# nebula-beta/MonocularSfM

Hardware: AMD Instinct MI355X
Metric: descriptor-pairs/sec (and image-pairs/sec); match-index bit-parity vs CPU (higher is better)
Workload: dtype f32

## Files before the change

monocularsfm_amd/csrc/msfm_batch.hip.h:

```cpp
#pragma once
namespace {
struct Batch {
    std::vector<PairDesc> pairs;
    std::vector<PfPair> pf;
    std::vector<int> id1, id2;
    std::vector<int> item_base;
    size_t n_items = 0, items_per_xcd = 0;
    MsfmItemChunks chunks = {};
    long long rp_elems = 0, cp_elems = 0, kf_elems = 0, kr_elems = 0, out_elems = 0, cand_elems = 0;
    int max_npad = 0;
    int64_t desc_pairs = 0;
    int64_t algo_bytes = 0;
    MsfmRoute route;
    std::vector<CandList> dense_lists;
    std::vector<VerifyPair> verify_pairs;
};

void build_items(Batch& b, int path, const std::vector<char>* only = nullptr, std::vector<int>* base_out = nullptr,
                 MsfmItemChunks* chunks_out = nullptr, const std::vector<char>* idle = nullptr) {
    std::vector<int> order(b.pairs.size());
    for (size_t p = 0; p < order.size(); ++p) order[p] = (int)p;
    if (b.id2.size() == b.pairs.size())
        std::stable_sort(order.begin(), order.end(), [&](int x, int y) { return b.id2[(size_t)x] < b.id2[(size_t)y]; });
    std::vector<int>& base = base_out ? *base_out : b.item_base;
// ... 367 lines not shown

constexpr size_t kTotalsBytes = 160;
constexpr int kTotalsSweep2 = 8, kTotalsSpans = 16, kTotalsSweep1 = 24, kTotalsSweep1b = 32;
struct PrefilterLaunch {
    msfm_ctx* ctx;
    Batch& b;
    size_t ev_base;
    PruneParams prune;
    size_t P = 0;
    HostClock hc;
    const MsfmRoute& route;
    std::vector<PfPair> pfq, pf16;
    long long dense_cand = 0;
    std::vector<int> item_base16;
    MsfmItemChunks chunks16 = {};
    size_t per16 = 0;
    long long kn = 1;
    hipEvent_t e0 = nullptr, e1 = nullptr, e2 = nullptr, e3 = nullptr;
    dim3 block, mgrid;
    unsigned sweep_grid = 8;
    const PairDesc* dp = nullptr;
    const PfPair* dpf = nullptr;
    float* tuv = nullptr;
    unsigned* colmask = nullptr;
    size_t n_lists = 0;
    const CandList* dl = nullptr;
    CompactPlan cp;
    size_t G = 0, M = 0;
    long long rows_cap = 0, cand_cap = 0, items_cap = 0;
    const PlanPair* dpp = nullptr;
    PlanCounts pc = {};
    PlanOut po = {};

    PrefilterLaunch(msfm_ctx* c, Batch& batch, size_t ev, PruneParams pr) : ctx(c), b(batch), ev_base(ev), prune(pr), route(batch.route) {}

    int apply_route() {
        P = b.pairs.size();
        hc = HostClock();
        SC.pf_pending = PfPending{};
        assign_partials(b, 1, 4 * ctx->cu_count);
        SC.prof.demoted_pairs += route.demoted_pairs;
        SC.pf_pending.refine = route.kind == kRouteQ8Refine;
        dense_cand = 0;
        for (size_t p = 0; p < P; ++p) {
            b.pf[p].tu_off = b.pairs[p].kf_off;
            b.pf[p].tv_off = b.pairs[p].kr_off;
            b.pf[p].cand_off = 0;
            b.pf[p].cand_cap = 0;
            if (!route.compact() && b.pairs[p].valid && b.pf[p].use) {
                b.pf[p].cand_off = dense_cand;
                b.pf[p].cand_cap = 16 * (b.pairs[p].n1 + b.pairs[p].n2) + 2048;
                dense_cand += b.pf[p].cand_cap;
                SC.pf_pending.dense_swept += (long long)b.pairs[p].n1pad * b.pairs[p].n2;
            }
        }
        pfq.clear(), pf16.clear();
        if (route.q8()) pfq = b.pf;
        for (size_t p = 0; p < P && (route.kind == kRouteI8 || route.q8()); ++p) {
            if (!b.pairs[p].valid || !b.pf[p].use) continue;
            PfPair& pp = route.q8() ? pfq[p] : b.pf[p];
            pp.use = route.q8() ? route.twin[p] : 1;
            if (!pp.use) continue;
            const Image &ia = ctx->images[b.id1[p]], &ib = ctx->images[b.id2[p]];
            pp.i8 = 1;
            if (route.q8()) {
                pp.a_h = reinterpret_cast<const _Float16*>(ia.q8);
                pp.b_h = reinterpret_cast<const _Float16*>(ib.q8);
// ... 334 lines not shown
                           SC.d_items.as<WorkItem>(), (float*)nullptr, (float*)nullptr, (float*)nullptr, (float*)nullptr,
                           (const float*)tuv, (const float*)tuv, SC.d_cand.as<int2>(), SC.d_cand_count.as<unsigned long long>(),
                           (const int*)nullptr, (int)b.n_items, (int*)nullptr, MsfmItemChunks{});
        HIPCHK(ctx, hipGetLastError());
        DBGSYNC(ctx, "sweep_kernel<2>");
        SC.prof.sweep2_launches += 1;
        HIPCHK(ctx, hipEventRecord(e3, SC.stream));
        HIPCHK(ctx, hipEventRecord(SC.sweep2_done, SC.stream));
        SC.sweep2_recorded = true;
        dl = SC.d_lists.as<CandList>();
        return MSFM_OK;
    }

    int launch_exact_and_finalize() {
        if (n_lists > 0) {
            const int wgs_per_xcd = std::max(1, ctx->cu_count / 8) * 8;
            const dim3 cgrid((unsigned)(8 * wgs_per_xcd));
            const unsigned long long* dcount = SC.d_cand_count.as<unsigned long long>();
#define MSFM_LAUNCH_EXACT(O)                                                                                             \
        hipLaunchKernelGGL(pf_exact_candidates_kernel<O>, cgrid, dim3(kExSpan), 0, SC.stream, dp, dl, dcount,                  \
                           (const int2*)SC.d_cand.as<int2>(), SC.d_best.as<unsigned long long>(), SC.d_second.as<unsigned long long>(), \
                           (int)n_lists, SC.d_totals.as<int>() + kTotalsSpans, (const int*)SC.d_cand_val.as<int>(), 0)
            if (route.kind == kRouteI8) MSFM_LAUNCH_EXACT(4);
            else if (ctx->order == MSFM_ORDER_SSE4X4) MSFM_LAUNCH_EXACT(0);
            else if (ctx->order == MSFM_ORDER_AVX2_FMA) MSFM_LAUNCH_EXACT(1);
            else MSFM_LAUNCH_EXACT(3);
#undef MSFM_LAUNCH_EXACT
            HIPCHK(ctx, hipGetLastError());
            DBGSYNC(ctx, "pf_exact_candidates_kernel");
    }
    if (!SC.keys_epilogue) {
        hipLaunchKernelGGL(pf_finalize_kernel, mgrid, dim3(256), 0, SC.stream, dp, dpf, (const float*)tuv, SC.d_best.as<unsigned long long>(),
                           SC.d_second.as<unsigned long long>(), SC.d_k_i0.as<int>(), SC.d_k_d0.as<float>(),
                           SC.d_k_d1.as<float>(), SC.d_fix_count.as<int>(), SC.d_fix_list.as<int4>(), SC.fix_cap_eff);
        HIPCHK(ctx, hipGetLastError());
        DBGSYNC(ctx, "pf_finalize_kernel");
    }
    if (n_lists > 0) {
        hipLaunchKernelGGL(pf_overflow_kernel, dim3((unsigned)((n_lists + 255) / 256)), dim3(256), 0, SC.stream, dl, (int)n_lists,
                           (const unsigned long long*)SC.d_cand_count.as<unsigned long long>(), (const PlanGroup*)SC.d_groups.as<PlanGroup>(),
                           (const int*)SC.d_gmembers.as<int>(), (const int*)SC.d_member_pair.as<int>(),
                           SC.d_overflow.as<unsigned char>(), SC.d_totals.as<unsigned long long>());
        HIPCHK(ctx, hipGetLastError());
    }
    SC.pf_pending.active = true;
    SC.pf_pending.n_lists = n_lists;
    SC.pf_pending.P = P;
    SC.pf_pending.ev_base = ev_base;
    hc.lap("launch sweep 2 .. finalize");
    return MSFM_OK;
    }

    int run() {
        int rc = apply_route();
        if (rc != MSFM_OK) return rc;
        rc = build_and_upload();
        if (rc != MSFM_OK || b.n_items == 0) return rc;
        rc = launch_sweep1();
        if (rc != MSFM_OK) return rc;
        if (route.compact()) {
            rc = plan_buffers();
            if (rc == MSFM_OK && route.q8()) rc = launch_route_q();
            if (rc == MSFM_OK) rc = launch_compact_sweep2();
        } else {
            rc = launch_dense_sweep2();
        }
        if (rc != MSFM_OK) return rc;
// ... 259 lines not shown
```

monocularsfm_amd/csrc/msfm_hostutil.h:

```cpp
#pragma once
#include <vector>

#if defined(__HIPCC__)
#include <hip/hip_runtime.h>
#define MSFM_HD __host__ __device__ inline __attribute__((always_inline))
#else
#define MSFM_HD inline
#endif

MSFM_HD int msfm_cp_pack(int hi, bool hi_valid, int lo, bool lo_valid) {
    unsigned c = 255u;
    if (lo_valid) {
        const unsigned x = (unsigned)(hi - lo) + 16u;
        int e = 27 - __builtin_clz(x);
        unsigned m = (x + (1u << e) - 1u) >> e;
        e += (int)(m >> 5);
        m = (m >> 5) ? 16u : m;
        const unsigned code = ((unsigned)e << 4) | (m - 16u);
        c = code >= 255u ? 255u : code;
    }
    return hi_valid ? (int)(((unsigned)hi << 8) | c) : (int)0x80000000;
}
constexpr int kCpNone = -(1 << 23);
MSFM_HD int msfm_cp_hi(int code) { return code >> 8; }
MSFM_HD bool msfm_cp_has_second(int code) { return (code & 255) != 255; }
MSFM_HD int msfm_cp_gap(int code) { const int c = code & 255; return ((16 + (c & 15)) << (c >> 4)) - 16; }

inline std::vector<long long> msfm_pipeline_marks(long long total, long long n_sub, double taper) {
    std::vector<long long> marks;
    if (n_sub < 2) return marks;
    const double last = taper, first = 2.0 - last;
    double acc = 0.0;
    marks.push_back(0);
// ... 192 lines not shown
    const long long rows_min = (hinted ? h_rows + h_rows / 8 : prior) + slack;
    MsfmPlanRoom r;
    r.hinted = hinted;
    r.rows = have_rows >= rows_min ? have_rows : mx(h_rows + h_rows / 2, prior) + slack;
    const long long cand_min = mx(8 * rows_min + 2048 * groups, h_cand);
    r.cand = have_cand >= cand_min ? have_cand : mx(8 * r.rows + 2048 * groups, h_cand);
    const long long items_min = mx(2 * ((rows_min / wg_rows + groups) * max_ranges + 64) / 8 * 8, (h_items + 64) / 8 * 8);
    r.items = have_items >= items_min ? have_items : mx(2 * ((r.rows / wg_rows + groups) * max_ranges + 64) / 8 * 8, (h_items + 64) / 8 * 8);
    return r;
}

inline unsigned long long msfm_pinned_piece_end(unsigned long long off) {
    const unsigned long long piece = 32ull << 20;
    if (off >= piece) return (off / piece + 1) * piece;
    unsigned long long end = 1ull << 20;
    while (end <= off) end *= 2;
    return end;
}

template <class AtomicMin>
MSFM_HD void msfm_fold_key(unsigned long long* best, unsigned long long* second, unsigned long long key, unsigned long long seen_best,
                           unsigned long long seen_second, AtomicMin amin) {
    if (key == seen_best) return;
    unsigned long long loser = key;
    if (key < seen_best) {
        const unsigned long long old = amin(best, key);
        if (old == key) return;
        loser = old > key ? old : key;
        if (loser == ~0ull) return;
    }
    if (loser < seen_second) (void)amin(second, loser);
}

MSFM_HD bool msfm_select_homography(int n_epipolar, int n_homography, double h_ratio) {
    return n_epipolar > 0 && (double)n_homography >= h_ratio * (double)n_epipolar;
}

MSFM_HD bool msfm_initial_candidate(int n_triangulated, double median_tri_angle, double mean_tri_angle, double mean_residual,
                                    int min_num_inliers, double tri_max_error, double tri_min_angle) {
    return n_triangulated >= min_num_inliers && median_tri_angle >= tri_min_angle && mean_tri_angle >= tri_min_angle &&
           mean_residual <= tri_max_error;
}
```

monocularsfm_amd/csrc/msfm_job.hip.h:

```cpp
#pragma once

static int call_prologue(msfm_ctx* ctx) {
    HIPCHK(ctx, hipSetDevice(ctx->device));
    ctx->cur = &ctx->sc[0];
    for (Scratch& s : ctx->sc) forget_sweeps(ctx, s);
    if (!ctx->deferred.empty()) {
        HIPCHK(ctx, hipDeviceSynchronize());
        ctx->deferred.flush();
    }
    return settle_store(ctx);
}

template <class Attempt>
static int rerun_alone(msfm_ctx* ctx, Attempt attempt) {
    for (int k = 1;; ++k) {
        bool retry = false;
        const int rc = attempt(&retry);
        if (rc != MSFM_OK || !retry) return rc;
        if (k >= 6) return fail(ctx, MSFM_E_DEVICE, "batch kept overflowing its queues");
    }
}

struct MatchJob {
    msfm_ctx* ctx = nullptr;
// ... 151 lines not shown
            w.b.pairs.push_back(pd);
            w.b.pf.push_back(pp);
            w.b.id1.push_back(pairs[2 * end]);
            w.b.id2.push_back(pairs[2 * end + 1]);
            ++end;
        }
        w.end = end;
        cost_done = cost_begin + cost;
        return prepare_batch_images(ctx, w.b, prune);
    }

    int issue(SubBatch& w, size_t ev_base) {
        Batch& b = w.b;
        const size_t P = b.pairs.size();
        const int begin = w.begin;
        w.ev_base = ev_base;
        w.exact_launched = false;
        SC.prof = msfm_profile{};
        SC.seq = ctx->issue_seq++;
        SC.sweep2_recorded = false;
        int rc = run_knn(ctx, b, ev_base, &w.exact_launched, prune, need_fix, true);
        if (rc != MSFM_OK) return rc;
        const long long oe = std::max<long long>(1, b.out_elems);
        HIPCHK(ctx, SC.d_st_qt.ensure(oe * sizeof(int2)));
        HIPCHK(ctx, SC.d_st_d.ensure(oe * 4));
        HIPCHK(ctx, SC.d_sub_qt.ensure(oe * sizeof(int2)));
        HIPCHK(ctx, SC.d_sub_d.ensure(oe * 4));
        HIPCHK(ctx, SC.d_counts.ensure(P * 4));
        HIPCHK(ctx, SC.d_sens.ensure(P * 4));
        HIPCHK(ctx, SC.d_offsets.ensure((P + 1) * 8));
        EpiParams ep = {prm.ratio, prm.cross_check, prm.max_distance};
        if (SC.keys_epilogue)
            hipLaunchKernelGGL(epilogue_kernel<KnnFromKeys>, dim3((unsigned)P), dim3(256), 0, SC.stream, SC.d_pairs.as<PairDesc>(), ep,
                               KnnFromKeys{SC.d_tu.as<float>(), SC.d_best.as<unsigned long long>(), SC.d_second.as<unsigned long long>()},
                               SC.d_st_qt.as<int2>(), SC.d_st_d.as<float>(), SC.d_counts.as<int>(), SC.d_sens.as<int>());
        else
            hipLaunchKernelGGL(epilogue_kernel<KnnFromArrays>, dim3((unsigned)P), dim3(256), 0, SC.stream, SC.d_pairs.as<PairDesc>(), ep,
                               KnnFromArrays{SC.d_k_i0.as<int>(), SC.d_k_d0.as<float>(), SC.d_k_d1.as<float>()},
                               SC.d_st_qt.as<int2>(), SC.d_st_d.as<float>(), SC.d_counts.as<int>(), SC.d_sens.as<int>());
        HIPCHK(ctx, hipGetLastError());
        const int* d_counts = SC.d_counts.as<int>();
        const int2* d_st_qt = SC.d_st_qt.as<int2>();
        const float* d_st_d = SC.d_st_d.as<float>();
        if (verify) {
            rc = issue_verify(b, begin, oe, ev_base);
            if (rc != MSFM_OK) return rc;
            d_counts = SC.d_counts2.as<int>();
            d_st_qt = SC.d_st2_qt.as<int2>();
            d_st_d = SC.d_st2_d.as<float>();
        }
        hipLaunchKernelGGL(scan_counts_kernel, dim3(1), dim3(256), 0, SC.stream, d_counts,
                           SC.d_offsets.as<long long>(), (int)P);
        HIPCHK(ctx, hipGetLastError());
        hipLaunchKernelGGL(gather_kernel, dim3((unsigned)P), dim3(256), 0, SC.stream, SC.d_pairs.as<PairDesc>(),
                           d_counts, SC.d_offsets.as<long long>(), d_st_qt,
                           d_st_d, SC.d_sub_qt.as<int2>(), SC.d_sub_d.as<float>());
        HIPCHK(ctx, hipGetLastError());
        rc = queue_tail_copies(ctx, P, select ? &SC.d_vs_records : nullptr);
        if (rc != MSFM_OK) return rc;
        if (pose) {
            HIPCHK(ctx, SC.h_tv.ensure(P * sizeof(msfm_two_view_record) + 64, 0));
            char* h = nullptr;
            HIPCHK(ctx, hipHostGetDevicePointer((void**)&h, SC.h_tv.p, 0));
            ExportSegs segs = {};
            segs.s[0] = ExportSeg{SC.d_tv_records.as<char>(), h, (unsigned)(P * sizeof(msfm_two_view_record))};
            hipLaunchKernelGGL(export_tail_kernel, dim3(32), dim3(256), 0, SC.stream, segs);
            HIPCHK(ctx, hipGetLastError());
// ... 372 lines not shown
```

monocularsfm_amd/csrc/msfm_kernels.hip.h:

```cpp
#pragma once
#include <hip/hip_runtime.h>
#include <stdint.h>

#pragma clang fp contract(off)

namespace msfm {

constexpr int kDim = 128;
constexpr int kBM = 128;
constexpr int kBN = 128;
constexpr int kTM = 8;
constexpr int kTN = 4;
constexpr int kThreads = 512;
constexpr int kChunkPos = 32;
constexpr int kChunks = kDim / kChunkPos;
constexpr int kPanelFloats = kBM * kDim;
constexpr int kSlotFloats = kChunkPos * kBN;
constexpr int kWaveCols = kBN / 8;
constexpr int kWaveSlotFloats = kChunkPos * kWaveCols;
constexpr int kLdsA = 0;
constexpr int kLdsB = kPanelFloats;
constexpr int kLdsFloats = kLdsB + 8 * 2 * kWaveSlotFloats;
constexpr int kLdsBytes = kLdsFloats * 4;

constexpr int kLdsBytesIdxStash = kLdsBytes + kTM * kThreads * 4;
template <int ORDER> struct OrderTraits;
template <> struct OrderTraits<0> {
    static constexpr int kGroups = 4, kIters = 8, kGroupPos = 32;
    static constexpr bool kFused = false;
    __host__ __device__ static int pos_to_k(int pos) {
        const int g = pos >> 5, v = (pos >> 3) & 3, it = pos & 7;
        const int lane = (g == 0) ? 0 : (g == 1) ? 2 : (g == 2) ? 1 : 3;
        return 16 * it + 4 * v + lane;
    }
};
// ... 417 lines not shown
template <int ORDER>
__global__ void tie_fixup_kernel(const PairDesc* __restrict__ pairs, const int* __restrict__ fix_count,
                                 const int4* __restrict__ fix_list, int fix_cap,
                                 int* __restrict__ k_i0, const float* __restrict__ k_d0) {
    MSFM_TAIL_PRIO();
    const int nfix = min(*fix_count, fix_cap);
    for (int f = blockIdx.x; f < nfix; f += gridDim.x) {
        const int4 w = fix_list[f];
        const PairDesc pd = pairs[w.x];
        const bool fwd = (w.y == 0);
        const float* me = (fwd ? pd.a_rawp : pd.b_rawp) + (size_t)w.z * kDim;
        const float* other = fwd ? pd.b_rawp : pd.a_rawp;
        const int n_other = fwd ? pd.n2 : pd.n1;
        const long long ko = (fwd ? pd.kf_off : pd.kr_off) + w.z;
        const float d0 = k_d0[ko];
        int best = 0x7fffffff;
        for (int t = threadIdx.x; t < n_other; t += 64) {
            const float s = fwd ? l2sqr_rowmajor<ORDER>(me, other + (size_t)t * kDim)
                                : l2sqr_rowmajor<ORDER>(other + (size_t)t * kDim, me);
            if (sqrtf(s) == d0) { best = t; break; }
        }
#pragma unroll
        for (int m = 32; m >= 1; m >>= 1) best = min(best, __shfl_xor(best, m));
        if (threadIdx.x == 0 && best != 0x7fffffff) k_i0[ko] = best;
    }
}

struct EpiParams {
    float ratio;
    int cross_check;
    double max_distance;
};

constexpr double kOrderEps = 1.0e-5;

__device__ __forceinline__ bool order_sensitive(int i0, float d0, float d1, float ratio, double max_distance, bool forward) {
    if (i0 < 0 || !(d1 < 3.402823466e+38f)) return false;
    const double lo0 = (double)d0 * (1.0 - kOrderEps), hi0 = (double)d0 * (1.0 + kOrderEps);
    const double lo1 = (double)d1 * (1.0 - kOrderEps), hi1 = (double)d1 * (1.0 + kOrderEps);
    if (forward && lo0 > max_distance) return false;
    const bool pass = d0 < ratio * d1;
    bool certified;
    if (pass)
        certified = hi0 < (double)ratio * lo1 && hi0 < lo1 && (!forward || hi0 <= max_distance || lo0 > max_distance);
    else
        certified = lo0 >= (double)ratio * hi1;
    return !certified;
}

struct KnnFromArrays {
    const int* i0;
    const float* d0;
    const float* d1;
    __device__ __forceinline__ void get(long long slot, int& i, float& a, float& b) const {
        i = i0[slot];
        a = d0[slot];
        b = d1[slot];
    }
};
struct KnnFromKeys {
    const float* tuv;
    const unsigned long long* best;
    const unsigned long long* second;
    __device__ __forceinline__ void get(long long slot, int& i, float& a, float& b) const {
        i = -1;
        a = b = 3.402823466e+38f;
        if (tuv[slot] == -f_inf()) return;
        const unsigned long long kb = best[slot], ks = second[slot];
        if (kb != ~0ull) { i = (int)(unsigned)(kb & 0xffffffffu); a = sqrtf(__uint_as_float((unsigned)(kb >> 32))); }
        if (ks != ~0ull) b = sqrtf(__uint_as_float((unsigned)(ks >> 32)));
    }
};

template <class KNN>
__global__ __launch_bounds__(256) void epilogue_kernel(const PairDesc* __restrict__ pairs, EpiParams prm, KNN knn,
                                                       int2* __restrict__ st_qt, float* __restrict__ st_d,
                                                       int* __restrict__ counts, int* __restrict__ sens_counts) {
    MSFM_TAIL_PRIO();
    const PairDesc pd = pairs[blockIdx.x];
    __shared__ int wsum[4];
    __shared__ int running, n_sens;
    if (threadIdx.x == 0) { running = 0; n_sens = 0; }
    __syncthreads();
    if (!pd.valid || pd.n2 < 2 || (prm.cross_check && pd.n1 < 2)) {
        if (threadIdx.x == 0) { counts[blockIdx.x] = 0; sens_counts[blockIdx.x] = 0; }
        return;
    }
    const bool certify = !pd.exact_int;
    const int lane = threadIdx.x & 63, wave = threadIdx.x >> 6;
    for (int q0 = 0; q0 < pd.n1; q0 += 256) {
        const int q = q0 + threadIdx.x;
        bool keep = false, sens = false;
        int t = -1;
        float d0 = 0.f;
        if (q < pd.n1) {
            float d1;
            knn.get(pd.kf_off + q, t, d0, d1);
            keep = (t >= 0) && (d1 < 3.402823466e+38f) && (d0 < prm.ratio * d1);
            sens = certify && order_sensitive(t, d0, d1, prm.ratio, prm.max_distance, true);
            if (keep && prm.cross_check) {
                int rq;
                float rd0, rd1;
                knn.get(pd.kr_off + t, rq, rd0, rd1);
                const bool rkeep = (rq >= 0) && (rd1 < 3.402823466e+38f) && (rd0 < prm.ratio * rd1);
                const int vis = rkeep ? rq : 0;
                keep = (vis == q);
            }
            if (keep && ((double)d0 > prm.max_distance)) keep = false;
        }
        const unsigned long long sb = __ballot(sens);
        if (lane == 0 && sb) atomicAdd(&n_sens, __popcll(sb));
        const unsigned long long bal = __ballot(keep);
        const int before = __popcll(bal & ((1ull << lane) - 1ull));
        if (lane == 0) wsum[wave] = __popcll(bal);
        __syncthreads();
        int off = running;
        for (int w = 0; w < wave; ++w) off += wsum[w];
        if (keep) {
            st_qt[pd.out_off + off + before] = make_int2(q, t);
            st_d[pd.out_off + off + before] = d0;
        }
        __syncthreads();
        if (threadIdx.x == 0) running += wsum[0] + wsum[1] + wsum[2] + wsum[3];
        __syncthreads();
    }
    if (certify && prm.cross_check)
        for (int t0 = 0; t0 < pd.n2; t0 += 256) {
            const int t = t0 + threadIdx.x;
            int ri = -1;
            float rd0 = 0.f, rd1 = 0.f;
            if (t < pd.n2) knn.get(pd.kr_off + t, ri, rd0, rd1);
            const bool s = t < pd.n2 && order_sensitive(ri, rd0, rd1, prm.ratio, prm.max_distance, false);
            const unsigned long long sb = __ballot(s);
            if (lane == 0 && sb) atomicAdd(&n_sens, __popcll(sb));
        }
    __syncthreads();
    if (threadIdx.x == 0) { counts[blockIdx.x] = running; sens_counts[blockIdx.x] = n_sens; }
}

__global__ void scan_counts_kernel(const int* __restrict__ counts, long long* __restrict__ offsets, int n) {
    MSFM_TAIL_PRIO();
    __shared__ long long carry;
    __shared__ long long wtot[4];
    if (threadIdx.x == 0) carry = 0;
    __syncthreads();
    const int lane = threadIdx.x & 63, wave = threadIdx.x >> 6;
    for (int base = 0; base < n; base += 256) {
        const int i = base + threadIdx.x;
        long long v = (i < n) ? counts[i] : 0;
        long long incl = v;
#pragma unroll
        for (int m = 1; m < 64; m <<= 1) {
            const long long o = __shfl_up(incl, m);
            if (lane >= m) incl += o;
        }
        if (lane == 63) wtot[wave] = incl;
        __syncthreads();
        long long woff = carry;
        for (int w = 0; w < wave; ++w) woff += wtot[w];
        if (i < n) offsets[i] = woff + incl - v;
        __syncthreads();
        if (threadIdx.x == 0) carry += wtot[0] + wtot[1] + wtot[2] + wtot[3];
        __syncthreads();
    }
// ... 19 lines not shown
```

monocularsfm_amd/csrc/msfm_prefilter.hip.h:

```cpp
#pragma once
#include "msfm_kernels.hip.h"

namespace msfm {

constexpr float kEpsRel = 1.5e-3f;
constexpr float kEpsAbs = 1.0e-6f;
constexpr float kF16Safe = 6.0e4f;

constexpr int kPfRB = 2;
constexpr int kPfWaveRows = 32 * kPfRB;
constexpr int kPfWaves = 8;
constexpr int kPfWgRows = kPfWaves * kPfWaveRows;
constexpr int kPfThreads = 64 * kPfWaves;
constexpr int kPfBT = 64;
constexpr int kPfRowHalfs = 136;
constexpr int kPfRowBytes = kPfRowHalfs * 2;
constexpr int kPfTileBytes = kPfBT * kPfRowBytes;
constexpr int kPfTilePieces = kPfTileBytes / 1024;
constexpr int kPfRing = 4;
constexpr int kPfColClasses = 4;
constexpr int kPfCandBuf = 256;
constexpr int kPfLdsBytes = kPfRing * kPfTileBytes + kPfWaves * kPfRing * 64 * 4 + kPfWaves * kPfCandBuf * 8 +
                            2 * kPfBT * kPfColClasses * 4;
static_assert(kPfTileBytes % 1024 == 0 && kPfTilePieces == 17, "tile = 17 DMA pieces");
// ... 15 lines not shown
    int cand_cap;
    int use;
    int i8;
    int a_h0, b_h0;
    int pad;
    const float* a_err;
    const float* b_err;
    const int* a_n2;
    const int* b_n2;
};

__device__ __forceinline__ void glds_copy_bytes(const void* g, void* lds, int bytes, int tid, int nthreads) {
    const int wave = __builtin_amdgcn_readfirstlane(tid >> 6), lane = tid & 63;
    const char* gp = reinterpret_cast<const char*>(g);
    char* lp = reinterpret_cast<char*>(lds);
#pragma unroll 1
    for (int piece = wave; piece * 1024 < bytes; piece += nthreads / 64)
        __builtin_amdgcn_global_load_lds((const __attribute__((address_space(1))) void*)(gp + piece * 1024 + lane * 16),
                                         (__attribute__((address_space(3))) void*)(lp + piece * 1024), 16, 0, 0);
}

__device__ __forceinline__ void v2_merge(float& s0, float& s1, float b0, float b1) {
    s1 = fminf(fmaxf(s0, b0), fminf(s1, b1));
    s0 = fminf(s0, b0);
}

#include "msfm_sweep.hip.h"
#include "msfm_sweep_i8.hip.h"

struct PruneParams {
    int prune;
    float ratio;
    float max_distance;
};

__device__ __forceinline__ bool pf_dead(float s0, float s1, float nrm, float eps, float other_max, PruneParams pr) {
    if (!pr.prune) return false;
    const float tiny = 1e-5f * (fabsf(s0) + fabsf(s1) + nrm + other_max);
    const float s0lb = fmaxf(s0 - eps - tiny, 0.f);
    const float s1ub = s1 + eps + tiny;
    const float d0lb = sqrtf(s0lb) * (1.f - 1e-6f);
    const bool ratio_fails = pr.ratio > 0.f && d0lb >= pr.ratio * sqrtf(s1ub) * (1.f + 1e-5f);
    const bool too_far = d0lb > pr.max_distance * (1.f + 1e-5f);
    return ratio_fails || too_far;
}

struct PlanPair {
    int fwd_member;
    int rev_member0;
    int rev_bits;
    int pad;
};


struct PlanCounts {
    const PlanPair* pp_plan;
    const int* member_group;
    int* cnt;
    int* gtot;
};

__global__ void pf_thresholds_kernel(const PairDesc* __restrict__ pairs, const PfPair* __restrict__ pf,
                                     const float* __restrict__ rp_s0, const float* __restrict__ rp_s1,
                                     const float* __restrict__ cp_s0, unsigned* __restrict__ colmask,
                                     float* __restrict__ tu, float* __restrict__ tv, PruneParams pr, PlanCounts plan,
                                     int marked ) {
// ... 30 lines not shown
        const float na = ld_anrm;
        const float eps = pp.i8 ? kI8Eps : kEpsRel * (na + pp.b_nrm_max) + kEpsAbs * (sqrtf(na) + sqrtf(pp.b_nrm_max)) + eps_norm;
        const float slack = pp.i8 ? 2.f * eps : 2.f * eps + 1e-5f * (fabsf(s1) + na + pp.b_nrm_max);
        const bool live = (e < pd.n1) && !pf_dead(s0, s1, na, eps, pp.b_nrm_max, pr);
        tu[pp.tu_off + e] = live ? s1 + slack : -f_inf();
        row_live = live;
    }
    if (in_c && marked && ld_tv == -f_inf()) {
        if (colmask) colmask[pp.tv_off + e] = 0;
    } else if (in_c) {
        float s0 = f_inf(), s1 = f_inf();
        auto partial = [&](long long i) -> float2 { return pp.i8 ? i8_cp_unpack(cpk[i]) : cp2[i]; };
        float bmin[16];
        if (nb <= 16) {
#pragma unroll
            for (int p = 0; p < 16; ++p) {
                bmin[p] = f_inf();
                if (p < nb) {
                    const float2 m = partial16(p);
                    bmin[p] = -2.f * m.x;
                    v2_merge(s0, s1, -2.f * m.x, -2.f * m.y);
                }
            }
        } else {
            for (int p = 0; p < nb; ++p) {
                const float2 m = partial(pd.cp_off + (long long)p * pd.n2pad + e);
                v2_merge(s0, s1, -2.f * m.x, -2.f * m.y);
            }
        }
        const float nb_ = ld_bnrm;
        const float eps = pp.i8 ? kI8Eps : kEpsRel * (nb_ + pp.a_nrm_max) + kEpsAbs * (sqrtf(nb_) + sqrtf(pp.a_nrm_max)) + eps_norm;
        const float slack = pp.i8 ? 2.f * eps : 2.f * eps + 1e-5f * (fabsf(s1) + nb_ + pp.a_nrm_max);
        const bool live = (e < pd.n2) && !pf_dead(s0, s1, nb_, eps, pp.a_nrm_max, pr);
        const float T = live ? s1 + slack : -f_inf();
        tv[pp.tv_off + e] = T;
        if (colmask) {
            const int g = (nb + 31) / 32;
            unsigned mask = 0;
            if (live) {
                if (nb <= 16) {
#pragma unroll
                    for (int p = 0; p < 16; ++p)
                        if (p < nb && bmin[p] <= T) mask |= 1u << p;
                } else {
                    for (int p = 0; p < nb; ++p) {
                        const float smin = -2.f * partial(pd.cp_off + (long long)p * pd.n2pad + e).x;
                        if (smin <= T) mask |= 1u << (p / g);
                    }
                }
            }
            colmask[pp.tv_off + e] = mask;
            col_bits = mask;
        }
    }
    if (plan.pp_plan) {
        const PlanPair pl = plan.pp_plan[blockIdx.y];
        if (pl.fwd_member < 0) return;
        __shared__ int hist[33];
        if (threadIdx.x < 33) hist[threadIdx.x] = 0;
        __syncthreads();
        const unsigned long long rl = __ballot(row_live);
        if ((threadIdx.x & 63) == 0 && rl) atomicAdd(&hist[32], __popcll(rl));
        while (col_bits) {
            const int bit = __builtin_ctz(col_bits);
            col_bits &= col_bits - 1;
            atomicAdd(&hist[bit], 1);
        }
// ... 186 lines not shown
            bv0[0] = y0.x, bv0[1] = y0.y, bv0[2] = y0.z, bv0[3] = y0.w, bv0[4] = y1.x, bv0[5] = y1.y, bv0[6] = y1.z, bv0[7] = y1.w;
            av1[0] = z0.x, av1[1] = z0.y, av1[2] = z0.z, av1[3] = z0.w, av1[4] = z1.x, av1[5] = z1.y, av1[6] = z1.z, av1[7] = z1.w;
            bv1[0] = w0.x, bv1[1] = w0.y, bv1[2] = w0.z, bv1[3] = w0.w, bv1[4] = w1.x, bv1[5] = w1.y, bv1[6] = w1.z, bv1[7] = w1.w;
        }
        const float r0 = pf_exact_combine<ORDER>(av0, bv0);
        const float r1 = pf_exact_combine<ORDER>(av1, bv1);
        if (sub == 0) {
            s_res[k0] = r0;
            s_res[k1] = r1;
        }
    }
    if (tid == 0) s_g = g_next;
    __syncthreads();
    if (live) {
        const float res = ORDER == 4 ? s_int : s_res[tid];
        if (res < f_inf()) {
            if (L.mode != 2) pf_fold(best, second, slot_r, pf_key(res, qt.y), sb_r, ss_r);
            if (L.mode != 1) pf_fold(best, second, slot_c, pf_key(res, qt.x), sb_c, ss_c);
        }
    }
   }
    round_base += total;
  }
}

#include "msfm_plan.hip.h"
#include "msfm_q8.hip.h"
#include "msfm_store.hip.h"

__global__ void pf_finalize_kernel(const PairDesc* __restrict__ pairs, const PfPair* __restrict__ pf,
                                   const float* __restrict__ tuv,
                                   const unsigned long long* __restrict__ best, const unsigned long long* __restrict__ second,
                                   int* __restrict__ k_i0, float* __restrict__ k_d0, float* __restrict__ k_d1,
                                   int* __restrict__ fix_count, int4* __restrict__ fix_list, int fix_cap) {
    MSFM_TAIL_PRIO();
    const PairDesc pd = pairs[blockIdx.y];
    const PfPair pp = pf[blockIdx.y];
    if (!pd.valid || !pp.use) return;
    const int e = blockIdx.x * blockDim.x + threadIdx.x;
    for (int dir = 0; dir < 2; ++dir) {
        const int n = dir == 0 ? pd.n1 : pd.n2;
        if (e >= n) continue;
        const long long ko = (dir == 0 ? pd.kf_off : pd.kr_off) + e;
        const bool dead = tuv[ko] == -f_inf();
        const unsigned long long b = dead ? ~0ull : best[ko], s = dead ? ~0ull : second[ko];
        int i0 = -1;
        float d0 = 3.402823466e+38f, d1 = 3.402823466e+38f;
        if (b != ~0ull) { i0 = (int)(unsigned)(b & 0xffffffffu); d0 = sqrtf(__uint_as_float((unsigned)(b >> 32))); }
        if (s != ~0ull) d1 = sqrtf(__uint_as_float((unsigned)(s >> 32)));
        k_i0[ko] = i0;
        k_d0[ko] = d0;
        k_d1[ko] = d1;
        if (i0 >= 0 && d0 == d1) {
            const int slot = atomicAdd(fix_count, 1);
            if (slot < fix_cap) fix_list[slot] = make_int4((int)blockIdx.y, dir, e, 0);
        }
    }
}

}
```

monocularsfm_amd/csrc/msfm_q8.hip.h:

```cpp
#pragma once

constexpr float kQ8LevelStep = 1.f / 16.f;

__global__ void pf_prune_q8_kernel(const PairDesc* __restrict__ pairs, const PfPair* __restrict__ pf, const PfPair* __restrict__ pfq,
                                   const float* __restrict__ rp_s0, const float* __restrict__ rp_s1, const float* __restrict__ cp_s0,
                                   unsigned* __restrict__ colmask, float* __restrict__ tuv, PruneParams pr, PlanCounts plan,
                                   float inv, int direct) {
    MSFM_TAIL_PRIO();
    const PairDesc pd = pairs[blockIdx.y];
    const PfPair pp = pf[blockIdx.y];
    if (!pd.valid || !pp.use) return;
    const PfPair pq = pfq[blockIdx.y];
    if (!pq.use) return;
    const int e = blockIdx.x * blockDim.x + threadIdx.x;
    bool row_live = false;
    unsigned col_bits = 0;
    auto lower = [&](float s0, float err) -> float { return fmaxf(sqrtf(fmaxf(s0, 0.f)) * inv * (1.f - 1e-6f) - err, 0.f); };
    auto upper = [&](float s1, float err) -> float { return sqrtf(s1 + 2.f) * inv * (1.f + 1e-6f) + err; };
    auto dead = [&](float s0, float s1, float err) -> bool {
        const float l0 = lower(s0, err), u1 = upper(s1, err);
        const bool ratio_fails = pr.ratio > 0.f && l0 * (1.f - 1e-5f) >= pr.ratio * u1 * (1.f + 1e-5f);
        const bool too_far = l0 * (1.f - 1e-5f) > pr.max_distance * (1.f + 1e-5f);
        return ratio_fails || too_far;
    };
// ... 23 lines not shown
        bool live = e < pd.n1;
        const float err = live ? (ld_aerr + pq.b_c) * (1.f + 1e-6f) : 0.f;
        if (live) live = !dead(s0, s1, err);
        float T = live ? f_inf() : -f_inf();
        if (live && direct) T = threshold(upper(s1, err), ld_anrm, pp.b_nrm_max);
        tuv[pp.tu_off + e] = T;
        row_live = live;
    }
    if (in_c) {
        float s0 = f_inf(), s1 = f_inf();
        float bmin[16];
        if (nb <= 16) {
#pragma unroll
            for (int p = 0; p < 16; ++p) {
                float2 m = make_float2(-f_inf(), -f_inf());
                if (p < nb) m = i8_cp_unpack(ld_cp[p]);
                bmin[p] = -2.f * m.x;
                v2_merge(s0, s1, -2.f * m.x, -2.f * m.y);
            }
        } else {
            for (int p = 0; p < nb; ++p) {
                const float2 m = i8_cp_unpack(cpk[pd.cp_off + (long long)p * pd.n2pad + e]);
                v2_merge(s0, s1, -2.f * m.x, -2.f * m.y);
            }
        }
        bool live = e < pd.n2;
        const float err = live ? (ld_berr + pq.a_c) * (1.f + 1e-6f) : 0.f;
        if (live) live = !dead(s0, s1, err);
        const int g = (nb + 31) / 32, bits = (nb + g - 1) / g;
        if (!direct) {
            tuv[pp.tv_off + e] = live ? f_inf() : -f_inf();
            col_bits = live ? (bits >= 32 ? 0xffffffffu : ((1u << bits) - 1u)) : 0u;
        } else {
            const float u1 = live ? upper(s1, err) : 0.f;
            tuv[pp.tv_off + e] = live ? threshold(u1, ld_bnrm, pp.a_nrm_max) : -f_inf();
            if (live) {
                if (nb <= 16) {
#pragma unroll
                    for (int p = 0; p < 16; ++p)
                        if (p < nb && lower(bmin[p], err) * (1.f - 1e-5f) <= u1 * (1.f + 1e-5f)) col_bits |= 1u << p;
                } else {
                    for (int p = 0; p < nb; ++p) {
                        const float smin = -2.f * i8_cp_unpack(cpk[pd.cp_off + (long long)p * pd.n2pad + e]).x;
                        if (lower(smin, err) * (1.f - 1e-5f) <= u1 * (1.f + 1e-5f)) col_bits |= 1u << (p / g);
                    }
                }
            }
        }
        colmask[pp.tv_off + e] = col_bits;
    }
    if (plan.pp_plan) {
        const PlanPair pl = plan.pp_plan[blockIdx.y];
        if (pl.fwd_member < 0) return;
        __shared__ int hist[33];
        if (threadIdx.x < 33) hist[threadIdx.x] = 0;
        __syncthreads();
        const unsigned long long rl = __ballot(row_live);
        if ((threadIdx.x & 63) == 0 && rl) atomicAdd(&hist[32], __popcll(rl));
        if (!direct) {
            const unsigned long long cl = __ballot(col_bits != 0u);
            if ((threadIdx.x & 63) == 0 && cl) atomicAdd(&hist[0], __popcll(cl));
        } else {
            while (col_bits) {
                const int bit = __builtin_ctz(col_bits);
                col_bits &= col_bits - 1;
                atomicAdd(&hist[bit], 1);
            }
// ... 44 lines not shown
```

Before: 5720 billion.

## Tighten reverse-direction sweep thresholds with a Lowe ratio cap

After: 6276 billion (median of 6 runs). 1.1x the previous value.

```diff
diff --git a/monocularsfm_amd/csrc/msfm_batch.hip.h b/monocularsfm_amd/csrc/msfm_batch.hip.h
--- a/monocularsfm_amd/csrc/msfm_batch.hip.h
+++ b/monocularsfm_amd/csrc/msfm_batch.hip.h
@@ -423,7 +423,9 @@
     PlanCounts pc = {};
     PlanOut po = {};
 
-    PrefilterLaunch(msfm_ctx* c, Batch& batch, size_t ev, PruneParams pr) : ctx(c), b(batch), ev_base(ev), prune(pr), route(batch.route) {}
+    PrefilterLaunch(msfm_ctx* c, Batch& batch, size_t ev, PruneParams pr) : ctx(c), b(batch), ev_base(ev), prune(pr), route(batch.route) {
+        prune.cap = msfm_ratio_cap_on(pr.prune, pr.ratio) ? 1 : 0;
+    }
 
     int apply_route() {
         P = b.pairs.size();
@@ -824,7 +826,7 @@
     if (!SC.keys_epilogue) {
         hipLaunchKernelGGL(pf_finalize_kernel, mgrid, dim3(256), 0, SC.stream, dp, dpf, (const float*)tuv, SC.d_best.as<unsigned long long>(),
                            SC.d_second.as<unsigned long long>(), SC.d_k_i0.as<int>(), SC.d_k_d0.as<float>(),
-                           SC.d_k_d1.as<float>(), SC.d_fix_count.as<int>(), SC.d_fix_list.as<int4>(), SC.fix_cap_eff);
+                           SC.d_k_d1.as<float>(), SC.d_fix_count.as<int>(), SC.d_fix_list.as<int4>(), SC.fix_cap_eff, prune.cap);
         HIPCHK(ctx, hipGetLastError());
         DBGSYNC(ctx, "pf_finalize_kernel");
     }
diff --git a/monocularsfm_amd/csrc/msfm_hostutil.h b/monocularsfm_amd/csrc/msfm_hostutil.h
--- a/monocularsfm_amd/csrc/msfm_hostutil.h
+++ b/monocularsfm_amd/csrc/msfm_hostutil.h
@@ -1,4 +1,5 @@
 #pragma once
+#include <cmath>
 #include <vector>
 
 #if defined(__HIPCC__)
@@ -257,6 +258,44 @@
     if (loser < seen_second) (void)amin(second, loser);
 }
 
+constexpr double kOrderEps = 1.0e-5;
+constexpr float kNoNeighbour = 3.402823466e+38f;
+
+constexpr float kRatioCapMax = 0.9f;
+inline bool msfm_ratio_cap_on(int prune, float ratio) { return prune != 0 && ratio > 0.f && ratio <= kRatioCapMax; }
+
+MSFM_HD float msfm_ratio_cap_distance(float u0, float u1, float ratio) {
+    const float c = u0 / ratio * (1.f + 4.f * (float)kOrderEps);
+    return c < u1 ? c : u1;
+}
+
+MSFM_HD float msfm_ratio_cap_sweep(float s0, float eps, float norms, float ratio) {
+    const float tiny = 1e-5f * (fabsf(s0) + norms);
+    const float s0ub = fmaxf(s0 + eps + tiny, 0.f);
+    const float c = s0ub / (ratio * ratio) * (1.f + 1e-4f);
+    return c + eps + 1e-5f * (fabsf(c) + norms);
+}
+MSFM_HD float msfm_ratio_cap_sweep_i8(float s0, float eps, float ratio) {
+    return ceilf(fmaxf(s0 + eps, 0.f) / (ratio * ratio) * (1.f + 1e-4f)) + eps;
+}
+
+MSFM_HD bool msfm_order_sensitive(int i0, float d0, float d1, float ratio, double max_distance, bool forward) {
+    const bool no_violator = d1 == __builtin_huge_valf();
+    if (i0 < 0 || !(d1 < kNoNeighbour || no_violator)) return false;
+    const double lo0 = (double)d0 * (1.0 - kOrderEps), hi0 = (double)d0 * (1.0 + kOrderEps);
+    if (forward && lo0 > max_distance) return false;
+    const bool cut_certified = !forward || hi0 <= max_distance || lo0 > max_distance;
+    if (no_violator) return !cut_certified;
+    const double lo1 = (double)d1 * (1.0 - kOrderEps), hi1 = (double)d1 * (1.0 + kOrderEps);
+    const bool pass = d0 < ratio * d1;
+    bool certified;
+    if (pass)
+        certified = hi0 < (double)ratio * lo1 && hi0 < lo1 && cut_certified;
+    else
+        certified = lo0 >= (double)ratio * hi1;
+    return !certified;
+}
+
 MSFM_HD bool msfm_select_homography(int n_epipolar, int n_homography, double h_ratio) {
     return n_epipolar > 0 && (double)n_homography >= h_ratio * (double)n_epipolar;
 }
diff --git a/monocularsfm_amd/csrc/msfm_job.hip.h b/monocularsfm_amd/csrc/msfm_job.hip.h
--- a/monocularsfm_amd/csrc/msfm_job.hip.h
+++ b/monocularsfm_amd/csrc/msfm_job.hip.h
@@ -207,7 +207,8 @@
         EpiParams ep = {prm.ratio, prm.cross_check, prm.max_distance};
         if (SC.keys_epilogue)
             hipLaunchKernelGGL(epilogue_kernel<KnnFromKeys>, dim3((unsigned)P), dim3(256), 0, SC.stream, SC.d_pairs.as<PairDesc>(), ep,
-                               KnnFromKeys{SC.d_tu.as<float>(), SC.d_best.as<unsigned long long>(), SC.d_second.as<unsigned long long>()},
+                               KnnFromKeys{SC.d_tu.as<float>(), SC.d_best.as<unsigned long long>(), SC.d_second.as<unsigned long long>(),
+                                           msfm_ratio_cap_on(prune.prune, prune.ratio) ? 1 : 0},
                                SC.d_st_qt.as<int2>(), SC.d_st_d.as<float>(), SC.d_counts.as<int>(), SC.d_sens.as<int>());
         else
             hipLaunchKernelGGL(epilogue_kernel<KnnFromArrays>, dim3((unsigned)P), dim3(256), 0, SC.stream, SC.d_pairs.as<PairDesc>(), ep,
diff --git a/monocularsfm_amd/csrc/msfm_kernels.hip.h b/monocularsfm_amd/csrc/msfm_kernels.hip.h
--- a/monocularsfm_amd/csrc/msfm_kernels.hip.h
+++ b/monocularsfm_amd/csrc/msfm_kernels.hip.h
@@ -1,6 +1,7 @@
 #pragma once
 #include <hip/hip_runtime.h>
 #include <stdint.h>
+#include "msfm_hostutil.h"
 
 #pragma clang fp contract(off)
 
@@ -484,27 +485,18 @@
     double max_distance;
 };
 
-constexpr double kOrderEps = 1.0e-5;
-
 __device__ __forceinline__ bool order_sensitive(int i0, float d0, float d1, float ratio, double max_distance, bool forward) {
-    if (i0 < 0 || !(d1 < 3.402823466e+38f)) return false;
-    const double lo0 = (double)d0 * (1.0 - kOrderEps), hi0 = (double)d0 * (1.0 + kOrderEps);
-    const double lo1 = (double)d1 * (1.0 - kOrderEps), hi1 = (double)d1 * (1.0 + kOrderEps);
-    if (forward && lo0 > max_distance) return false;
-    const bool pass = d0 < ratio * d1;
-    bool certified;
-    if (pass)
-        certified = hi0 < (double)ratio * lo1 && hi0 < lo1 && (!forward || hi0 <= max_distance || lo0 > max_distance);
-    else
-        certified = lo0 >= (double)ratio * hi1;
-    return !certified;
+    return msfm_order_sensitive(i0, d0, d1, ratio, max_distance, forward);
+}
+__device__ __forceinline__ bool lowe_keep(int i0, float d0, float d1, float ratio) {
+    return (i0 >= 0) && (d1 < kNoNeighbour || d1 == f_inf()) && (d0 < ratio * d1);
 }
 
 struct KnnFromArrays {
     const int* i0;
     const float* d0;
     const float* d1;
-    __device__ __forceinline__ void get(long long slot, int& i, float& a, float& b) const {
+    __device__ __forceinline__ void get(long long slot, bool , int& i, float& a, float& b) const {
         i = i0[slot];
         a = d0[slot];
         b = d1[slot];
@@ -514,13 +506,15 @@
     const float* tuv;
     const unsigned long long* best;
     const unsigned long long* second;
-    __device__ __forceinline__ void get(long long slot, int& i, float& a, float& b) const {
+    int cap;
+    __device__ __forceinline__ void get(long long slot, bool reverse, int& i, float& a, float& b) const {
         i = -1;
-        a = b = 3.402823466e+38f;
+        a = b = kNoNeighbour;
         if (tuv[slot] == -f_inf()) return;
         const unsigned long long kb = best[slot], ks = second[slot];
         if (kb != ~0ull) { i = (int)(unsigned)(kb & 0xffffffffu); a = sqrtf(__uint_as_float((unsigned)(kb >> 32))); }
         if (ks != ~0ull) b = sqrtf(__uint_as_float((unsigned)(ks >> 32)));
+        else if (cap && reverse && kb != ~0ull) b = f_inf();
     }
 };
 
@@ -547,14 +541,14 @@
         float d0 = 0.f;
         if (q < pd.n1) {
             float d1;
-            knn.get(pd.kf_off + q, t, d0, d1);
-            keep = (t >= 0) && (d1 < 3.402823466e+38f) && (d0 < prm.ratio * d1);
+            knn.get(pd.kf_off + q, false, t, d0, d1);
+            keep = lowe_keep(t, d0, d1, prm.ratio);
             sens = certify && order_sensitive(t, d0, d1, prm.ratio, prm.max_distance, true);
             if (keep && prm.cross_check) {
                 int rq;
                 float rd0, rd1;
-                knn.get(pd.kr_off + t, rq, rd0, rd1);
-                const bool rkeep = (rq >= 0) && (rd1 < 3.402823466e+38f) && (rd0 < prm.ratio * rd1);
+                knn.get(pd.kr_off + t, true, rq, rd0, rd1);
+                const bool rkeep = lowe_keep(rq, rd0, rd1, prm.ratio);
                 const int vis = rkeep ? rq : 0;
                 keep = (vis == q);
             }
@@ -581,7 +575,7 @@
             const int t = t0 + threadIdx.x;
             int ri = -1;
             float rd0 = 0.f, rd1 = 0.f;
-            if (t < pd.n2) knn.get(pd.kr_off + t, ri, rd0, rd1);
+            if (t < pd.n2) knn.get(pd.kr_off + t, true, ri, rd0, rd1);
             const bool s = t < pd.n2 && order_sensitive(ri, rd0, rd1, prm.ratio, prm.max_distance, false);
             const unsigned long long sb = __ballot(s);
             if (lane == 0 && sb) atomicAdd(&n_sens, __popcll(sb));
diff --git a/monocularsfm_amd/csrc/msfm_prefilter.hip.h b/monocularsfm_amd/csrc/msfm_prefilter.hip.h
--- a/monocularsfm_amd/csrc/msfm_prefilter.hip.h
+++ b/monocularsfm_amd/csrc/msfm_prefilter.hip.h
@@ -71,6 +71,7 @@
     int prune;
     float ratio;
     float max_distance;
+    int cap;
 };
 
 __device__ __forceinline__ bool pf_dead(float s0, float s1, float nrm, float eps, float other_max, PruneParams pr) {
@@ -167,7 +168,9 @@
         const float eps = pp.i8 ? kI8Eps : kEpsRel * (nb_ + pp.a_nrm_max) + kEpsAbs * (sqrtf(nb_) + sqrtf(pp.a_nrm_max)) + eps_norm;
         const float slack = pp.i8 ? 2.f * eps : 2.f * eps + 1e-5f * (fabsf(s1) + nb_ + pp.a_nrm_max);
         const bool live = (e < pd.n2) && !pf_dead(s0, s1, nb_, eps, pp.a_nrm_max, pr);
-        const float T = live ? s1 + slack : -f_inf();
+        float T = live ? s1 + slack : -f_inf();
+        if (live && pr.cap)
+            T = fminf(T, pp.i8 ? msfm_ratio_cap_sweep_i8(s0, eps, pr.ratio) : msfm_ratio_cap_sweep(s0, eps, nb_ + pp.a_nrm_max, pr.ratio));
         tv[pp.tv_off + e] = T;
         if (colmask) {
             const int g = (nb + 31) / 32;
@@ -420,7 +423,8 @@
                                    const float* __restrict__ tuv,
                                    const unsigned long long* __restrict__ best, const unsigned long long* __restrict__ second,
                                    int* __restrict__ k_i0, float* __restrict__ k_d0, float* __restrict__ k_d1,
-                                   int* __restrict__ fix_count, int4* __restrict__ fix_list, int fix_cap) {
+                                   int* __restrict__ fix_count, int4* __restrict__ fix_list, int fix_cap,
+                                   int cap ) {
     MSFM_TAIL_PRIO();
     const PairDesc pd = pairs[blockIdx.y];
     const PfPair pp = pf[blockIdx.y];
@@ -436,6 +440,7 @@
         float d0 = 3.402823466e+38f, d1 = 3.402823466e+38f;
         if (b != ~0ull) { i0 = (int)(unsigned)(b & 0xffffffffu); d0 = sqrtf(__uint_as_float((unsigned)(b >> 32))); }
         if (s != ~0ull) d1 = sqrtf(__uint_as_float((unsigned)(s >> 32)));
+        else if (cap && dir == 1 && i0 >= 0) d1 = f_inf();
         k_i0[ko] = i0;
         k_d0[ko] = d0;
         k_d1[ko] = d1;
diff --git a/monocularsfm_amd/csrc/msfm_q8.hip.h b/monocularsfm_amd/csrc/msfm_q8.hip.h
--- a/monocularsfm_amd/csrc/msfm_q8.hip.h
+++ b/monocularsfm_amd/csrc/msfm_q8.hip.h
@@ -79,7 +79,8 @@
             tuv[pp.tv_off + e] = live ? f_inf() : -f_inf();
             col_bits = live ? (bits >= 32 ? 0xffffffffu : ((1u << bits) - 1u)) : 0u;
         } else {
-            const float u1 = live ? upper(s1, err) : 0.f;
+            float u1 = live ? upper(s1, err) : 0.f;
+            if (live && pr.cap) u1 = msfm_ratio_cap_distance(upper(s0, err), u1, pr.ratio);
             tuv[pp.tv_off + e] = live ? threshold(u1, ld_bnrm, pp.a_nrm_max) : -f_inf();
             if (live) {
                 if (nb <= 16) {
```
